# Runki2018/litehandnet

Hardware: AMD Instinct MI355X
Metric: images/sec fwd+bwd @256x256 bs64 litehandnet (higher is better)
Workload: dtype f32; 1 GPU; litehandnet variant B (MSRB hourglass litehourglass.py) C=128, 256x256x3 -> 21x64x64, per-GPU batch 64, train-mode BN, fwd + TopdownHeatmapLoss + bwd + fused Adam; global_batch=64, parallelism=dp1

## Files before the change

### litehandnet_amd/csrc/k_conv_stem.hip

```cpp
#include "lhn_common.h"

__global__ void __launch_bounds__(256) k_stem_fwd(const float* __restrict__ img, const float* __restrict__ w, lhn_view y,
                                                  double* __restrict__ stats, int Hi, int Wi, int K, int stride, int pad,
                                                  lhn_bnfin fin) {
  extern __shared__ __attribute__((aligned(16))) float smem[];
  const int CO = y.C, CG = CO >> 3, KK = K * K, T = 3 * KK;
  float* Ws = smem;
  float* red = smem + T * CO;
  const int tid = threadIdx.x;
  for (int i = tid; i < T * CO; i += 256) {
    const int co = i / T, t = i - co * T;
    Ws[t * CO + co] = w[i];
  }
  __syncthreads();
  const int cg = tid % CG, pl = tid / CG, PL = 256 / CG;
  const int64_t total = (int64_t)y.N * y.H * y.W;
  float s[8], q[8];
#pragma unroll
  for (int j = 0; j < 8; ++j) s[j] = q[j] = 0.f;
  for (int64_t pix = (int64_t)blockIdx.x * PL + pl; pix < total; pix += (int64_t)gridDim.x * PL) {
    const int wo = (int)(pix % y.W);
    const int64_t t = pix / y.W;
    const int ho = (int)(t % y.H), n = (int)(t / y.H);
    float acc[8];
#pragma unroll
    for (int j = 0; j < 8; ++j) acc[j] = 0.f;
    for (int c = 0; c < 3; ++c) {
      const float* plane = img + ((int64_t)n * 3 + c) * Hi * Wi;
      for (int kh = 0; kh < K; ++kh) {
        const int ih = ho * stride - pad + kh;
        if (ih < 0 || ih >= Hi) continue;
        for (int kw = 0; kw < K; ++kw) {
          const int iw = wo * stride - pad + kw;
          if (iw < 0 || iw >= Wi) continue;
          const float v = plane[(int64_t)ih * Wi + iw];
          const float* wr = Ws + (c * KK + kh * K + kw) * CO + cg * 8;
          const f4 w0 = *reinterpret_cast<const f4*>(wr), w1 = *reinterpret_cast<const f4*>(wr + 4);
          acc[0] += v * w0.x; acc[1] += v * w0.y; acc[2] += v * w0.z; acc[3] += v * w0.w;
          acc[4] += v * w1.x; acc[5] += v * w1.y; acc[6] += v * w1.z; acc[7] += v * w1.w;
        }
      }
    }
    float* o = y.data + pix * y.cstride + y.coff + cg * 8;
    *reinterpret_cast<f4*>(o) = (f4){acc[0], acc[1], acc[2], acc[3]};
    *reinterpret_cast<f4*>(o + 4) = (f4){acc[4], acc[5], acc[6], acc[7]};
#pragma unroll
    for (int j = 0; j < 8; ++j) {
      s[j] += acc[j];
      q[j] += acc[j] * acc[j];
    }
  }
  if (stats) {
#pragma unroll
    for (int j = 0; j < 8; ++j) {
      red[tid * 16 + j] = s[j];
      red[tid * 16 + 8 + j] = q[j];
    }
    __syncthreads();
    if (tid < CO) {
      const int g = tid >> 3, j = tid & 7;
      double sd = 0, qd = 0;
      for (int p = 0; p < PL; ++p) {
        sd += red[(p * CG + g) * 16 + j];
        qd += red[(p * CG + g) * 16 + 8 + j];
      }
      double* st = stats + (size_t)(blockIdx.x % LHN_STAT_REPLICAS) * 2 * CO;
      atomicAdd(st + tid, sd);
      atomicAdd(st + CO + tid, qd);
    }
    if (fin.counter && lhn_last_block(fin.counter)) lhn_bn_finalize_block(fin, stats);
  }
}


__global__ void __launch_bounds__(256) k_stem3_fwd_mfma(const float* __restrict__ img, const float* __restrict__ w, lhn_view y,
                                                        double* __restrict__ stats, int Hi, int Wi, int stride, int pad, lhn_bnfin fin) {
  constexpr int CO = 32, LDV = 36;
  __shared__ __attribute__((aligned(16))) float Vs[256 * LDV];
  __shared__ double redd[4][2 * CO];
  const int tid = threadIdx.x, lane = tid & 63, wave = __builtin_amdgcn_readfirstlane(tid >> 6), l31 = lane & 31, lh = lane >> 5;
  float wreg[16];
#pragma unroll
  for (int ks = 0; ks < 16; ++ks) {
    const int tap = 16 * lh + ks;
    wreg[ks] = tap < 27 ? w[l31 * 27 + tap] : 0.f;
  }
  for (int t = 27; t < 32; ++t) Vs[tid * LDV + t] = 0.f;
  const int64_t total = (int64_t)y.N * y.H * y.W;
  const int64_t ntiles = (total + 255) / 256;
  float v[27];
  auto issue = [&](int64_t tile) __attribute__((always_inline)) {
    const int64_t pix = tile * 256 + tid;
    const int64_t pc = pix < total ? pix : total - 1;
    const int wo = (int)(pc % y.W);
    const int64_t r = pc / y.W;
    const int ho = (int)(r % y.H), n = (int)(r / y.H);
#pragma unroll
    for (int c = 0; c < 3; ++c) {
      const float* plane = img + ((int64_t)n * 3 + c) * Hi * Wi;
#pragma unroll
      for (int kh = 0; kh < 3; ++kh) {
        const int ih = ho * stride - pad + kh, ihc = min(max(ih, 0), Hi - 1);
#pragma unroll
        for (int kw = 0; kw < 3; ++kw) {
          const int iw = wo * stride - pad + kw, iwc = min(max(iw, 0), Wi - 1);
          const float t = plane[(int64_t)ihc * Wi + iwc];
          v[c * 9 + kh * 3 + kw] = (ih == ihc && iw == iwc) ? t : 0.f;
        }
      }
    }
  };
  float s = 0.f, q = 0.f, kk = 0.f;
  int cnt = 0;
  int64_t tile = blockIdx.x;
  if (tile < ntiles) issue(tile);
  for (; tile < ntiles; tile += gridDim.x) {
    __syncthreads();
#pragma unroll
    for (int t = 0; t < 27; ++t) Vs[tid * LDV + t] = v[t];
    __syncthreads();
    if (tile + gridDim.x < ntiles) issue(tile + gridDim.x);
#pragma unroll
    for (int h = 0; h < 2; ++h) {
      const int prow = wave * 64 + 32 * h;
      const f4* ap = reinterpret_cast<const f4*>(Vs + (prow + l31) * LDV + 16 * lh);
      const f4 a0 = ap[0], a1 = ap[1], a2 = ap[2], a3 = ap[3];
      const float a[16] = {a0.x, a0.y, a0.z, a0.w, a1.x, a1.y, a1.z, a1.w, a2.x, a2.y, a2.z, a2.w, a3.x, a3.y, a3.z, a3.w};
      f16v acc;
#pragma unroll
      for (int r = 0; r < 16; ++r) acc[r] = 0.f;
#pragma unroll
      for (int ks = 0; ks < 16; ++ks) acc = __builtin_amdgcn_mfma_f32_32x32x2f32(a[ks], wreg[ks], acc, 0, 0, 0);
      const int64_t pbase = tile * 256 + prow + 4 * lh;
#pragma unroll
      for (int r = 0; r < 16; ++r) {
        const int64_t pix = pbase + (r & 3) + 8 * (r >> 2);
        if (pix < total) {
          y.data[pix * y.cstride + y.coff + l31] = acc[r];
          if (cnt == 0) kk = acc[r];
          const float d = acc[r] - kk;
          s += d;
          q += d * d;
          ++cnt;
        }
      }
    }
  }
  if (stats) {
    const double k0 = kk, c0 = cnt;
    double sd = (double)s + c0 * k0, qd = (double)q + 2.0 * k0 * (double)s + c0 * k0 * k0;
    sd += __shfl_xor(sd, 32, 64);
    qd += __shfl_xor(qd, 32, 64);
    if (lh == 0) {
      redd[wave][l31] = sd;
      redd[wave][CO + l31] = qd;
    }
    __syncthreads();
    if (tid < 2 * CO) {
      double* st = stats + (size_t)(blockIdx.x % LHN_STAT_REPLICAS) * 2 * CO;
      atomicAdd(st + tid, redd[0][tid] + redd[1][tid] + redd[2][tid] + redd[3][tid]);
    }
    if (fin.counter && lhn_last_block(fin.counter)) lhn_bn_finalize_block(fin, stats);
  }
}


__global__ void __launch_bounds__(256, 2) k_stem7_fwd_mfma(const float* __restrict__ img, const float* __restrict__ w, lhn_view y,
                                                        double* __restrict__ stats, int Hi, int Wi, int stride, int pad, lhn_bnfin fin) {
  constexpr int CO = 64, T = 147, TP = 160, NKS = TP / 2, LDV = TP + 4, BMP = 64, G = 4, NR = 6, NV = NR * 7;
  extern __shared__ __attribute__((aligned(16))) float smem[];
  float* Vs = smem;
  double* redd = reinterpret_cast<double*>(smem + BMP * LDV);
  const int tid = threadIdx.x, lane = tid & 63, wave = __builtin_amdgcn_readfirstlane(tid >> 6), l31 = lane & 31, lh = lane >> 5;
  const int cot = wave & 1, pg = wave >> 1, co = cot * 32 + l31;
  float wreg[NKS];
#pragma unroll
  for (int ks = 0; ks < NKS; ++ks) {
    const int tap = NKS * lh + ks;
    wreg[ks] = tap < T ? w[co * T + tap] : 0.f;
  }
  const int p = tid & (BMP - 1), g = tid >> 6;
  for (int t = T + g; t < TP; t += G) Vs[p * LDV + t] = 0.f;
  const int64_t total = (int64_t)y.N * y.H * y.W;
  const int64_t ntiles = (total + BMP - 1) / BMP;
  float v[NV];
  auto issue = [&](int64_t tile) __attribute__((always_inline)) {
    const int64_t pix = tile * BMP + p;
    const int64_t pc = pix < total ? pix : total - 1;
    const int wo = (int)(pc % y.W);
    const int64_t r = pc / y.W;
    const int ho = (int)(r % y.H), n = (int)(r / y.H);
    const float* base = img + (int64_t)n * 3 * Hi * Wi;
    const int iw0 = wo * stride - pad;
#pragma unroll
    for (int jr = 0; jr < NR; ++jr) {
      const int row = min(g + G * jr, 20), c = row / 7, kh = row - 7 * c;
      const int ih = ho * stride - pad + kh, ihc = min(max(ih, 0), Hi - 1);
      const float* rb = base + ((int64_t)c * Hi + ihc) * Wi;
#pragma unroll
      for (int kw = 0; kw < 7; ++kw) {
        const int iw = iw0 + kw, iwc = min(max(iw, 0), Wi - 1);
        const float q = rb[iwc];
        v[jr * 7 + kw] = (ih == ihc && iw == iwc) ? q : 0.f;
      }
    }
  };
  float s = 0.f, q = 0.f, kk = 0.f;
  int cnt = 0;
  int64_t tile = blockIdx.x;
  if (tile < ntiles) issue(tile);
  for (; tile < ntiles; tile += gridDim.x) {
    __syncthreads();
#pragma unroll
    for (int jr = 0; jr < NR; ++jr)
      if (g + G * jr < 21)
#pragma unroll
        for (int kw = 0; kw < 7; ++kw) Vs[p * LDV + (g + G * jr) * 7 + kw] = v[jr * 7 + kw];
    __syncthreads();
    if (tile + gridDim.x < ntiles) issue(tile + gridDim.x);
    const f4* ap = reinterpret_cast<const f4*>(Vs + (pg * 32 + l31) * LDV + NKS * lh);
    f16v acc;
#pragma unroll
    for (int r = 0; r < 16; ++r) acc[r] = 0.f;
#pragma unroll
    for (int c = 0; c < NKS / 4; ++c) {
      if ((c & 3) == 0) asm volatile("" ::: "memory");
      const f4 a = ap[c];
      acc = __builtin_amdgcn_mfma_f32_32x32x2f32(a.x, wreg[4 * c + 0], acc, 0, 0, 0);
      acc = __builtin_amdgcn_mfma_f32_32x32x2f32(a.y, wreg[4 * c + 1], acc, 0, 0, 0);
      acc = __builtin_amdgcn_mfma_f32_32x32x2f32(a.z, wreg[4 * c + 2], acc, 0, 0, 0);
      acc = __builtin_amdgcn_mfma_f32_32x32x2f32(a.w, wreg[4 * c + 3], acc, 0, 0, 0);
    }
    const int64_t pbase = tile * BMP + pg * 32 + 4 * lh;
#pragma unroll
    for (int r = 0; r < 16; ++r) {
      const int64_t pix = pbase + (r & 3) + 8 * (r >> 2);
      if (pix < total) {
        y.data[pix * y.cstride + y.coff + co] = acc[r];
        if (cnt == 0) kk = acc[r];
        const float d = acc[r] - kk;
        s += d;
        q += d * d;
        ++cnt;
      }
    }
  }
  if (stats) {
    const double k0 = kk, c0 = cnt;
    double sd = (double)s + c0 * k0, qd = (double)q + 2.0 * k0 * (double)s + c0 * k0 * k0;
    sd += __shfl_xor(sd, 32, 64);
    qd += __shfl_xor(qd, 32, 64);
    __syncthreads();
    if (lh == 0) {
      redd[pg * 2 * CO + co] = sd;
      redd[pg * 2 * CO + CO + co] = qd;
    }
    __syncthreads();
    if (tid < 2 * CO) {
      double* st = stats + (size_t)(blockIdx.x % LHN_STAT_REPLICAS) * 2 * CO;
      atomicAdd(st + tid, redd[tid] + redd[2 * CO + tid]);
    }
    if (fin.counter && lhn_last_block(fin.counter)) lhn_bn_finalize_block(fin, stats);
  }
}

extern "C" int lhn_conv_stem_fwd(const float* img, const float* w, const lhn_view* y, double* stats, int Hi, int Wi, int k,
                                 int stride, int pad, const lhn_bnfin* finp, void* stream) {
  lhn_bnfin fin;
  if (finp && stats) fin = *finp; else fin.counter = nullptr;
  LHN_CHECK_ARG(img && w && lhn_view_ok(y), "lhn_conv_stem_fwd: bad view / null pointer");
  LHN_CHECK_ARG(y->C % 8 == 0 && pow2(y->C / 8) && y->C <= 256, "lhn_conv_stem_fwd: Cout=%d", y->C);
  LHN_CHECK_ARG((k == 1 || k == 3 || k == 5 || k == 7) && stride >= 1, "lhn_conv_stem_fwd: k=%d", k);
  const int Ho = (Hi + 2 * pad - k) / stride + 1, Wo = (Wi + 2 * pad - k) / stride + 1;
  LHN_CHECK_ARG(y->H == Ho && y->W == Wo, "lhn_conv_stem_fwd: output %dx%d, expected %dx%d", y->H, y->W, Ho, Wo);
  const int PL = 256 / (y->C / 8);
  const size_t lds = (size_t)(3 * k * k * y->C) * 4 + 256 * 16 * 4;
  const bool mfma = !lhn_dw_force_gather() && ((k == 7 && y->C == 64) || (k == 3 && y->C == 32));
  LHN_CHECK_ARG(mfma || lds <= 65536, "lhn_conv_stem_fwd: k=%d Cout=%d needs %zu B of LDS (limit 65536 B)", k, y->C, lds);
  if (k == 7 && y->C == 64 && !lhn_dw_force_gather()) {
    const size_t lds7 = (size_t)64 * 164 * 4 + 2 * 2 * 64 * 8;
    static LhnKernelCfg cfg7;
    int per_cu = 1;
    if (!lhn_kernel_cfg(cfg7, &k_stem7_fwd_mfma, lds7, 3, &per_cu)) {
      lhn_set_error("lhn_conv_stem_fwd: cannot reserve %zu B of LDS", lds7);
      return 2;
    }
    const int64_t ntiles = ((int64_t)y->N * Ho * Wo + 63) / 64;
    int grid = lhn_num_cus() * per_cu;
    if (grid > ntiles) grid = (int)ntiles;
    hipLaunchKernelGGL(k_stem7_fwd_mfma, dim3(grid), dim3(256), lds7, (hipStream_t)stream, img, w, *y, stats, Hi, Wi, stride, pad, fin);
  } else if (k == 3 && y->C == 32 && !lhn_dw_force_gather()) {
    hipLaunchKernelGGL(k_stem3_fwd_mfma, dim3(grid_for((int64_t)y->N * Ho * Wo, 256, 3)), dim3(256), 0, (hipStream_t)stream, img, w, *y,
                       stats, Hi, Wi, stride, pad, fin);
  } else
    hipLaunchKernelGGL(k_stem_fwd, dim3(grid_for((int64_t)y->N * Ho * Wo, PL, 8)), dim3(256), lds, (hipStream_t)stream, img,
                       w, *y, stats, Hi, Wi, k, stride, pad, fin);
  LHN_CHECK_LAUNCH("lhn_conv_stem_fwd");
  return 0;
}

__device__ __forceinline__ f4 dw_load_dy(const lhn_view& y, const lhn_gradview& g, const Xf4& xf, const Gr4& gr,
                                         int64_t pix, int n, int h, int w, int ca) {
  const f4 raw = *reinterpret_cast<const f4*>(y.data + pix * y.cstride + ca);
  const f4 dz = *reinterpret_cast<const f4*>(g.dz + pix * y.cstride + ca);
  const f4 du = lhn_grad_du(y, g, xf, raw, dz, n, h, w, ca);
  return gr.A * du + gr.B * raw + gr.Cc;
}

template <int K, int KR>
__global__ void __launch_bounds__(256) k_stem_bwd(const float* __restrict__ img, lhn_view y, lhn_gradview gy,
                                                  float* __restrict__ dw, int Hi, int Wi, int stride, int pad, int nrep,
                                                  int64_t rep_stride, int kh0) {
  dw += (size_t)(blockIdx.x % nrep) * rep_stride;
  constexpr int T = 3 * KR * K;
  __shared__ f4 red[256];
  const int C4 = y.C >> 2;
  const int tid = threadIdx.x, c4 = tid % C4, pl = tid / C4, PL = 256 / C4;
  const int cy = y.coff + 4 * c4;
  const Xf4 yxf = lhn_load_xf(y, cy);
  const Gr4 ygr = lhn_load_coef(gy, y.cstride, cy);
  f4 acc[T];
#pragma unroll
  for (int i = 0; i < T; ++i) acc[i] = (f4){0.f, 0.f, 0.f, 0.f};
  const int64_t total = (int64_t)y.N * y.H * y.W;
  for (int64_t pix = (int64_t)blockIdx.x * PL + pl; pix < total; pix += (int64_t)gridDim.x * PL) {
    const int wo = (int)(pix % y.W);
    const int64_t t = pix / y.W;
    const int ho = (int)(t % y.H), n = (int)(t / y.H);
    const f4 dy = dw_load_dy(y, gy, yxf, ygr, pix, n, ho, wo, cy);
#pragma unroll
    for (int c = 0; c < 3; ++c) {
      const float* plane = img + ((int64_t)n * 3 + c) * Hi * Wi;
#pragma unroll
      for (int r = 0; r < KR; ++r) {
        const int ih = ho * stride - pad + kh0 + r;
#pragma unroll
        for (int kw = 0; kw < K; ++kw) {
          const int iw = wo * stride - pad + kw;
          float v = 0.f;
          if (ih >= 0 && ih < Hi && iw >= 0 && iw < Wi) v = plane[(int64_t)ih * Wi + iw];
          acc[(c * KR + r) * K + kw] += dy * v;
        }
      }
    }
  }
  constexpr int TW = 3 * K * K;
#pragma unroll
  for (int i = 0; i < T; ++i) {
    __syncthreads();
    red[tid] = acc[i];
    __syncthreads();
    if (tid < C4) {
      f4 s = (f4){0.f, 0.f, 0.f, 0.f};
      for (int j = 0; j < PL; ++j) s += red[j * C4 + tid];
      const int c = i / (KR * K), r = (i / K) % KR, kw = i % K, e = c * K * K + (kh0 + r) * K + kw;
      atomicAdd(dw + (4 * tid + 0) * TW + e, s.x);
      atomicAdd(dw + (4 * tid + 1) * TW + e, s.y);
      atomicAdd(dw + (4 * tid + 2) * TW + e, s.z);
      atomicAdd(dw + (4 * tid + 3) * TW + e, s.w);
    }
  }
}


__global__ void __launch_bounds__(256) k_stem3_bwd_mfma(const float* __restrict__ img, lhn_view y, lhn_gradview gy, float* __restrict__ dw,
                                                        int Hi, int Wi, int stride, int pad, int nrep, int64_t rep_stride) {
  constexpr int CO = 32, LDY = CO + 4, LDV = 33;
  extern __shared__ __attribute__((aligned(16))) float smem[];
  float* dYs = smem;
  float* Vs = smem + 256 * LDY;
  const int tid = threadIdx.x, lane = tid & 63, wave = __builtin_amdgcn_readfirstlane(tid >> 6), l31 = lane & 31, lh = lane >> 5;
  const int c4 = tid & 7, prow = tid >> 3;
  const int cy = y.coff + 4 * c4;
  const Xf4 yxf = lhn_load_xf(y, cy);
  const Gr4 ygr = lhn_load_coef(gy, y.cstride, cy);
  for (int t = 27; t < 32; ++t) Vs[tid * LDV + t] = 0.f;
  f16v acc;
#pragma unroll
  for (int r = 0; r < 16; ++r) acc[r] = 0.f;
  const int64_t total = (int64_t)y.N * y.H * y.W;
  const int64_t ntiles = (total + 255) / 256;
  f4 yraw[8], zraw[8];
  float v[27];
  auto issue = [&](int64_t tile) __attribute__((always_inline)) {
#pragma unroll
    for (int j = 0; j < 8; ++j) {
      int64_t pix = tile * 256 + prow + 32 * j;
      pix = pix < total ? pix : total - 1;
      yraw[j] = *reinterpret_cast<const f4*>(y.data + pix * y.cstride + cy);
      zraw[j] = *reinterpret_cast<const f4*>(gy.dz + pix * y.cstride + cy);
    }
    const int64_t pix = tile * 256 + tid;
    const int64_t pc = pix < total ? pix : total - 1;
    const int wo = (int)(pc % y.W);
    const int64_t r = pc / y.W;
    const int ho = (int)(r % y.H), n = (int)(r / y.H);
#pragma unroll
    for (int c = 0; c < 3; ++c) {
      const float* plane = img + ((int64_t)n * 3 + c) * Hi * Wi;
#pragma unroll
      for (int kh = 0; kh < 3; ++kh) {
        const int ih = ho * stride - pad + kh, ihc = min(max(ih, 0), Hi - 1);
#pragma unroll
        for (int kw = 0; kw < 3; ++kw) {
          const int iw = wo * stride - pad + kw, iwc = min(max(iw, 0), Wi - 1);
          const float t = plane[(int64_t)ihc * Wi + iwc];
          v[c * 9 + kh * 3 + kw] = (ih == ihc && iw == iwc) ? t : 0.f;
        }
      }
    }
  };
  int64_t tile = blockIdx.x;
  if (tile < ntiles) issue(tile);
  for (; tile < ntiles; tile += gridDim.x) {
    __syncthreads();
#pragma unroll
    for (int j = 0; j < 8; ++j) {
      const int p = prow + 32 * j;
      const int64_t pix = tile * 256 + p;
      f4 d = (f4){0.f, 0.f, 0.f, 0.f};
      if (pix < total) {
        const int wo = (int)(pix % y.W);
        const int64_t r = pix / y.W;
        const f4 du = lhn_grad_du(y, gy, yxf, yraw[j], zraw[j], (int)(r / y.H), (int)(r % y.H), wo, cy);
        d = ygr.A * du + ygr.B * yraw[j] + ygr.Cc;
      }
      *reinterpret_cast<f4*>(dYs + p * LDY + 4 * c4) = d;
    }
#pragma unroll
    for (int t = 0; t < 27; ++t) Vs[tid * LDV + t] = v[t];
    __syncthreads();
    if (tile + gridDim.x < ntiles) issue(tile + gridDim.x);
    const float* ar = dYs + (wave * 64 + lh) * LDY + l31;
    const float* br = Vs + (wave * 64 + lh) * LDV + l31;
#pragma unroll 8
    for (int ks = 0; ks < 32; ++ks) acc = __builtin_amdgcn_mfma_f32_32x32x2f32(ar[2 * ks * LDY], br[2 * ks * LDV], acc, 0, 0, 0);
  }
  __syncthreads();
  float* part = dYs;
#pragma unroll
  for (int r = 0; r < 16; ++r) part[(wave * 16 + r) * 64 + lane] = acc[r];
  __syncthreads();
  dw += (size_t)(blockIdx.x % nrep) * rep_stride;
  for (int i = tid; i < CO * 27; i += 256) {
    const int co = i / 27, t = i - co * 27;
    const int r = (co & 3) + 4 * (co >> 3), ln = t + 32 * ((co >> 2) & 1);
    const float v = part[(0 * 16 + r) * 64 + ln] + part[(1 * 16 + r) * 64 + ln] + part[(2 * 16 + r) * 64 + ln] + part[(3 * 16 + r) * 64 + ln];
    atomicAdd(dw + i, v);
  }
}


__global__ void __launch_bounds__(256, 2) k_stem7_bwd_mfma(const float* __restrict__ img, lhn_view y, lhn_gradview gy, float* __restrict__ dw,
                                                           int Hi, int Wi, int stride, int pad, int nrep, int64_t rep_stride) {
  constexpr int CO = 64, T = 147, LDY = CO + 4, LDV = 161, BMP = 64, G = 4, NR = 6;
  extern __shared__ __attribute__((aligned(16))) float smem[];
  float* dYs = smem;
  float* Vs = smem + BMP * LDY;
  const int tid = threadIdx.x, lane = tid & 63, wave = __builtin_amdgcn_readfirstlane(tid >> 6), l31 = lane & 31, lh = lane >> 5;
  const int c4 = tid & 15, prow = tid >> 4;
  const int cy = y.coff + 4 * c4;
  const Xf4 yxf = lhn_load_xf(y, cy);
  const Gr4 ygr = lhn_load_coef(gy, y.cstride, cy);
  const int p = tid & (BMP - 1), g = tid >> 6;
  for (int t = T + g; t < 160; t += G) Vs[p * LDV + t] = 0.f;
  f16v acc[3];
#pragma unroll
  for (int i = 0; i < 3; ++i)
#pragma unroll
    for (int r = 0; r < 16; ++r) acc[i][r] = 0.f;
  const int64_t total = (int64_t)y.N * y.H * y.W;
  const int64_t ntiles = (total + BMP - 1) / BMP;
  f4 yraw[4], zraw[4];
  float v[NR * 7];
  auto issue = [&](int64_t tile) __attribute__((always_inline)) {
#pragma unroll
    for (int j = 0; j < 4; ++j) {
      int64_t pix = tile * BMP + prow + 16 * j;
      pix = pix < total ? pix : total - 1;
      yraw[j] = *reinterpret_cast<const f4*>(y.data + pix * y.cstride + cy);
      zraw[j] = *reinterpret_cast<const f4*>(gy.dz + pix * y.cstride + cy);
    }
    const int64_t pix = tile * BMP + p;
    const int64_t pc = pix < total ? pix : total - 1;
    const int wo = (int)(pc % y.W);
    const int64_t r = pc / y.W;
    const int ho = (int)(r % y.H), n = (int)(r / y.H);
    const float* base = img + (int64_t)n * 3 * Hi * Wi;
    const int iw0 = wo * stride - pad;
#pragma unroll
    for (int jr = 0; jr < NR; ++jr) {
      const int row = min(g + G * jr, 20), c = row / 7, kh = row - 7 * c;
      const int ih = ho * stride - pad + kh, ihc = min(max(ih, 0), Hi - 1);
      const float* rb = base + ((int64_t)c * Hi + ihc) * Wi;
#pragma unroll
      for (int kw = 0; kw < 7; ++kw) {
        const int iw = iw0 + kw, iwc = min(max(iw, 0), Wi - 1);
        const float q = rb[iwc];
        v[jr * 7 + kw] = (ih == ihc && iw == iwc) ? q : 0.f;
      }
    }
  };
  int64_t tile = blockIdx.x;
  if (tile < ntiles) issue(tile);
  for (; tile < ntiles; tile += gridDim.x) {
    __syncthreads();
#pragma unroll
    for (int j = 0; j < 4; ++j) {
      const int pp = prow + 16 * j;
      const int64_t pix = tile * BMP + pp;
      f4 d = (f4){0.f, 0.f, 0.f, 0.f};
      if (pix < total) {
        const int wo = (int)(pix % y.W);
        const int64_t r = pix / y.W;
        const f4 du = lhn_grad_du(y, gy, yxf, yraw[j], zraw[j], (int)(r / y.H), (int)(r % y.H), wo, cy);
        d = ygr.A * du + ygr.B * yraw[j] + ygr.Cc;
      }
      *reinterpret_cast<f4*>(dYs + pp * LDY + 4 * c4) = d;
    }
#pragma unroll
    for (int jr = 0; jr < NR; ++jr)
      if (g + G * jr < 21)
#pragma unroll
        for (int kw = 0; kw < 7; ++kw) Vs[p * LDV + (g + G * jr) * 7 + kw] = v[jr * 7 + kw];
    __syncthreads();
    if (tile + gridDim.x < ntiles) issue(tile + gridDim.x);
#pragma unroll
    for (int i = 0; i < 3; ++i) {
      const int job = wave + 4 * i;
      if (job < 10) {
        const float* ar = dYs + lh * LDY + (job & 1) * 32 + l31;
        const float* br = Vs + lh * LDV + (job >> 1) * 32 + l31;
#pragma unroll 8
        for (int ks = 0; ks < 32; ++ks) acc[i] = __builtin_amdgcn_mfma_f32_32x32x2f32(ar[2 * ks * LDY], br[2 * ks * LDV], acc[i], 0, 0, 0);
      }
    }
  }
  dw += (size_t)(blockIdx.x % nrep) * rep_stride;
#pragma unroll
  for (int i = 0; i < 3; ++i) {
    const int job = wave + 4 * i;
    if (job < 10) {
      const int t = (job >> 1) * 32 + l31;
#pragma unroll
      for (int r = 0; r < 16; ++r) {
        const int co = (job & 1) * 32 + (r & 3) + 8 * (r >> 2) + 4 * lh;
        if (t < T) atomicAdd(dw + co * T + t, acc[i][r]);
      }
    }
  }
}

extern "C" int lhn_conv_stem_bwd(const float* img, const lhn_view* y, const lhn_gradview* gy, float* dw, int Hi, int Wi, int k,
                                 int stride, int pad, int nrep, int64_t rep_stride, void* stream) {
  if (nrep < 1) nrep = 1;
  LHN_CHECK_ARG(img && lhn_view_ok(y) && gy && gy->dz && dw, "lhn_conv_stem_bwd: bad view / null pointer");
  LHN_CHECK_ARG(pow2(y->C / 4) && y->C <= 256 && (k == 1 || k == 3 || k == 7), "lhn_conv_stem_bwd: Cout=%d k=%d", y->C, k);
  const int PL = 256 / (y->C / 4);
  const int g = grid_for((int64_t)y->N * y->H * y->W, PL, 4);
  if (k == 7 && y->C == 64 && !lhn_dw_force_gather()) {
    const size_t lds = (size_t)64 * (68 + 161) * 4;
    static LhnKernelCfg cfg7;
    int per_cu = 1;
    if (!lhn_kernel_cfg(cfg7, &k_stem7_bwd_mfma, lds, 2, &per_cu)) {
      lhn_set_error("lhn_conv_stem_bwd: cannot reserve %zu B of LDS", lds);
      return 2;
    }
    const int64_t ntiles = ((int64_t)y->N * y->H * y->W + 63) / 64;
    int grid = lhn_num_cus() * per_cu;
    if (grid > ntiles) grid = (int)ntiles;
    hipLaunchKernelGGL(k_stem7_bwd_mfma, dim3(grid), dim3(256), lds, (hipStream_t)stream, img, *y, *gy, dw, Hi, Wi, stride, pad, nrep, rep_stride);
  } else if (k == 3 && y->C == 32 && !lhn_dw_force_gather()) {
    const size_t lds = (size_t)256 * (36 + 33) * 4;
    static LhnKernelCfg cfg;
    int per_cu = 1;
    if (!lhn_kernel_cfg(cfg, &k_stem3_bwd_mfma, lds, 2, &per_cu)) {
      lhn_set_error("lhn_conv_stem_bwd: cannot reserve %zu B of LDS", lds);
      return 2;
    }
    const int64_t ntiles = ((int64_t)y->N * y->H * y->W + 255) / 256;
    int grid = lhn_num_cus() * per_cu;
    if (grid > ntiles) grid = (int)ntiles;
    hipLaunchKernelGGL(k_stem3_bwd_mfma, dim3(grid), dim3(256), lds, (hipStream_t)stream, img, *y, *gy, dw, Hi, Wi, stride, pad, nrep, rep_stride);
  } else if (k == 3)
    hipLaunchKernelGGL((k_stem_bwd<3, 3>), dim3(g), dim3(256), 0, (hipStream_t)stream, img, *y, *gy, dw, Hi, Wi, stride, pad, nrep, rep_stride, 0);
  else if (k == 1)
    hipLaunchKernelGGL((k_stem_bwd<1, 1>), dim3(g), dim3(256), 0, (hipStream_t)stream, img, *y, *gy, dw, Hi, Wi, stride, pad, nrep, rep_stride, 0);
  else
    for (int kh = 0; kh < 7; ++kh)
      hipLaunchKernelGGL((k_stem_bwd<7, 1>), dim3(g), dim3(256), 0, (hipStream_t)stream, img, *y, *gy, dw, Hi, Wi, stride, pad, nrep, rep_stride, kh);
  LHN_CHECK_LAUNCH("lhn_conv_stem_bwd");
  return 0;
}
```

Baseline: 9508 images/s.

## Add per-wave tiled stem3 conv fwd/bwd kernels with double-buffered gathers

Adds new 3x3 stem conv forward and backward MFMA kernels in which each wave owns 32-pixel tiles. Image gathers are double-buffered in registers and prefetched while the current tile's MFMAs run, and pixel indices are advanced incrementally instead of recomputed with divisions. The backward kernel uses per-wave LDS slices with wave barriers instead of block-wide syncs, and has a template variant that skips gate/pool index math when those are absent. The path is on by default, can be disabled with an env var, and is limited to inputs under 2^30 elements because offsets are 32-bit.

```diff
diff --git a/litehandnet_amd/csrc/k_conv_stem.hip b/litehandnet_amd/csrc/k_conv_stem.hip
--- a/litehandnet_amd/csrc/k_conv_stem.hip
+++ b/litehandnet_amd/csrc/k_conv_stem.hip
@@ -145,6 +145,149 @@
         }
       }
     }
+  }
+  if (stats) {
+    const double k0 = kk, c0 = cnt;
+    double sd = (double)s + c0 * k0, qd = (double)q + 2.0 * k0 * (double)s + c0 * k0 * k0;
+    sd += __shfl_xor(sd, 32, 64);
+    qd += __shfl_xor(qd, 32, 64);
+    if (lh == 0) {
+      redd[wave][l31] = sd;
+      redd[wave][CO + l31] = qd;
+    }
+    __syncthreads();
+    if (tid < 2 * CO) {
+      double* st = stats + (size_t)(blockIdx.x % LHN_STAT_REPLICAS) * 2 * CO;
+      atomicAdd(st + tid, redd[0][tid] + redd[1][tid] + redd[2][tid] + redd[3][tid]);
+    }
+    if (fin.counter && lhn_last_block(fin.counter)) lhn_bn_finalize_block(fin, stats);
+  }
+}
+
+
+struct Stem3Pix {
+  int n, ho, wo, dn[2], dh[2], dw[2];
+  __device__ __forceinline__ void init(int64_t p, int64_t step0, int64_t step1, int H, int W) {
+    wo = (int)(p % W);
+    int64_t r = p / W;
+    ho = (int)(r % H), n = (int)(r / H);
+    dw[0] = (int)(step0 % W);
+    r = step0 / W;
+    dh[0] = (int)(r % H), dn[0] = (int)(r / H);
+    dw[1] = (int)(step1 % W);
+    r = step1 / W;
+    dh[1] = (int)(r % H), dn[1] = (int)(r / H);
+  }
+  __device__ __forceinline__ void advance(int H, int W, int i) {
+    wo += dw[i];
+    int c = wo >= W;
+    wo -= c ? W : 0;
+    ho += dh[i] + c;
+    c = ho >= H;
+    ho -= c ? H : 0;
+    n += dn[i] + c;
+  }
+};
+__device__ __forceinline__ void stem3_gather(const float* __restrict__ img, int n, int ho, int wo, int lh, int Hi, int Wi, int stride,
+                                             int pad, float (&v)[16], unsigned& mask) {
+  const int HW = Hi * Wi, base = n * 3 * HW;
+  int ro[3], cl[3];
+  unsigned rok = 0, cok = 0;
+#pragma unroll
+  for (int k = 0; k < 3; ++k) {
+    const int ih = ho * stride - pad + k, ihc = min(max(ih, 0), Hi - 1);
+    const int iw = wo * stride - pad + k, iwc = min(max(iw, 0), Wi - 1);
+    ro[k] = ihc * Wi;
+    cl[k] = iwc;
+    rok |= (unsigned)(ih == ihc) << k;
+    cok |= (unsigned)(iw == iwc) << k;
+  }
+  unsigned m = 0;
+#pragma unroll
+  for (int ks = 0; ks < 16; ++ks) {
+    const int t0 = ks, t1 = 16 + ks < 27 ? 16 + ks : ks;
+    const int o0 = (t0 / 9) * HW + ro[(t0 % 9) / 3] + cl[t0 % 3], o1 = (t1 / 9) * HW + ro[(t1 % 9) / 3] + cl[t1 % 3];
+    const unsigned k0 = (rok >> ((t0 % 9) / 3)) & (cok >> (t0 % 3)) & 1u;
+    const unsigned k1 = 16 + ks < 27 ? ((rok >> ((t1 % 9) / 3)) & (cok >> (t1 % 3)) & 1u) : 0u;
+    v[ks] = *reinterpret_cast<const float*>(reinterpret_cast<const char*>(img) + (unsigned)(base + (lh ? o1 : o0)) * 4u);
+    m |= (lh ? k1 : k0) << ks;
+  }
+  mask = m;
+}
+static bool stem3_wave_tiles_on(int N, int Hi, int Wi) {
+  static int v = -1;
+  if (v < 0) {
+    const char* e = getenv("LHN_STEM3_WAVE_TILES");
+    v = (e && e[0] == '0') ? 0 : 1;
+  }
+  return v != 0 && (int64_t)N * 3 * Hi * Wi < ((int64_t)1 << 30);
+}
+
+__global__ void __launch_bounds__(256, 4) k_stem3_fwd_mfma_wt(const float* __restrict__ img, const float* __restrict__ w, lhn_view y,
+                                                           double* __restrict__ stats, int Hi, int Wi, int stride, int pad, lhn_bnfin fin) {
+  constexpr int CO = 32;
+  __shared__ double redd[4][2 * CO];
+  const int tid = threadIdx.x, lane = tid & 63, wave = __builtin_amdgcn_readfirstlane(tid >> 6), l31 = lane & 31, lh = lane >> 5;
+  float wreg[16];
+#pragma unroll
+  for (int ks = 0; ks < 16; ++ks) {
+    const int tap = 16 * lh + ks;
+    wreg[ks] = tap < 27 ? w[l31 * 27 + tap] : 0.f;
+  }
+  const int64_t total = (int64_t)y.N * y.H * y.W;
+  const int64_t nblk = (total + 255) / 256, G = gridDim.x;
+  Stem3Pix px;
+  px.init(((int64_t)blockIdx.x * 8 + 2 * wave) * 32 + l31, 32, (8 * G - 1) * 32, y.H, y.W);
+  float va[16], vb[16];
+  unsigned ma = 0, mb = 0;
+  auto issue = [&](float (&v)[16], unsigned& m, int second) __attribute__((always_inline)) {
+    stem3_gather(img, min(px.n, y.N - 1), px.ho, px.wo, lh, Hi, Wi, stride, pad, v, m);
+    px.advance(y.H, y.W, second);
+  };
+  float s = 0.f, q = 0.f, kk = 0.f;
+  int cnt = 0;
+  const unsigned voff = (unsigned)(4 * lh * y.cstride + l31) * 4u;
+  auto tile_of = [&](float (&v)[16], unsigned& m, int64_t tile, bool more, int second) __attribute__((always_inline)) {
+    f16v acc;
+#pragma unroll
+    for (int r = 0; r < 16; ++r) acc[r] = 0.f;
+#pragma unroll
+    for (int ks = 0; ks < 16; ++ks) acc = __builtin_amdgcn_mfma_f32_32x32x2f32(((m >> ks) & 1u) ? v[ks] : 0.f, wreg[ks], acc, 0, 0, 0);
+    if (more) issue(v, m, second);
+    char* const ybase = reinterpret_cast<char*>(y.data + tile * 32 * y.cstride + y.coff);
+    const int left = (int)max((int64_t)0, min((int64_t)32, total - tile * 32));
+    if (left == 32) {
+#pragma unroll
+      for (int r = 0; r < 16; ++r) {
+        *reinterpret_cast<float*>(ybase + (size_t)((r & 3) + 8 * (r >> 2)) * y.cstride * 4 + voff) = acc[r];
+        if (cnt == 0) kk = acc[r];
+        const float d = acc[r] - kk;
+        s += d;
+        q += d * d;
+        ++cnt;
+      }
+    } else {
+#pragma unroll
+      for (int r = 0; r < 16; ++r)
+        if (4 * lh + (r & 3) + 8 * (r >> 2) < left) {
+          *reinterpret_cast<float*>(ybase + (size_t)((r & 3) + 8 * (r >> 2)) * y.cstride * 4 + voff) = acc[r];
+          if (cnt == 0) kk = acc[r];
+          const float d = acc[r] - kk;
+          s += d;
+          q += d * d;
+          ++cnt;
+        }
+    }
+  };
+  int64_t T = blockIdx.x;
+  if (T < nblk) {
+    issue(va, ma, 0);
+    issue(vb, mb, 1);
+  }
+  for (; T < nblk; T += G) {
+    const bool more = T + G < nblk;
+    tile_of(va, ma, T * 8 + 2 * wave, more, 0);
+    tile_of(vb, mb, T * 8 + 2 * wave + 1, more, 1);
   }
   if (stats) {
     const double k0 = kk, c0 = cnt;
@@ -290,8 +433,12 @@
     if (grid > ntiles) grid = (int)ntiles;
     hipLaunchKernelGGL(k_stem7_fwd_mfma, dim3(grid), dim3(256), lds7, (hipStream_t)stream, img, w, *y, stats, Hi, Wi, stride, pad, fin);
   } else if (k == 3 && y->C == 32 && !lhn_dw_force_gather()) {
-    hipLaunchKernelGGL(k_stem3_fwd_mfma, dim3(grid_for((int64_t)y->N * Ho * Wo, 256, 3)), dim3(256), 0, (hipStream_t)stream, img, w, *y,
-                       stats, Hi, Wi, stride, pad, fin);
+    if (stem3_wave_tiles_on(y->N, Hi, Wi)) {
+      hipLaunchKernelGGL(k_stem3_fwd_mfma_wt, dim3(grid_for((int64_t)y->N * Ho * Wo, 256, 3)), dim3(256), 0, (hipStream_t)stream, img, w, *y,
+                         stats, Hi, Wi, stride, pad, fin);
+    } else
+      hipLaunchKernelGGL(k_stem3_fwd_mfma, dim3(grid_for((int64_t)y->N * Ho * Wo, 256, 3)), dim3(256), 0, (hipStream_t)stream, img, w, *y,
+                         stats, Hi, Wi, stride, pad, fin);
   } else
     hipLaunchKernelGGL(k_stem_fwd, dim3(grid_for((int64_t)y->N * Ho * Wo, PL, 8)), dim3(256), lds, (hipStream_t)stream, img,
                        w, *y, stats, Hi, Wi, k, stride, pad, fin);
@@ -438,6 +585,103 @@
   }
   __syncthreads();
   float* part = dYs;
+#pragma unroll
+  for (int r = 0; r < 16; ++r) part[(wave * 16 + r) * 64 + lane] = acc[r];
+  __syncthreads();
+  dw += (size_t)(blockIdx.x % nrep) * rep_stride;
+  for (int i = tid; i < CO * 27; i += 256) {
+    const int co = i / 27, t = i - co * 27;
+    const int r = (co & 3) + 4 * (co >> 3), ln = t + 32 * ((co >> 2) & 1);
+    const float v = part[(0 * 16 + r) * 64 + ln] + part[(1 * 16 + r) * 64 + ln] + part[(2 * 16 + r) * 64 + ln] + part[(3 * 16 + r) * 64 + ln];
+    atomicAdd(dw + i, v);
+  }
+}
+
+
+template <bool GP>
+__global__ void __launch_bounds__(256, 2) k_stem3_bwd_mfma_wt(const float* __restrict__ img, lhn_view y, lhn_gradview gy, float* __restrict__ dw,
+                                                           int Hi, int Wi, int stride, int pad, int nrep, int64_t rep_stride) {
+  if constexpr (!GP) {
+    y.gate = nullptr;
+    gy.dpool = nullptr;
+  }
+  constexpr int CO = 32, LDY = CO + 4, LDV = 33, WS = 32 * (LDY + LDV);
+  extern __shared__ __attribute__((aligned(16))) float smem[];
+  const int tid = threadIdx.x, lane = tid & 63, wave = __builtin_amdgcn_readfirstlane(tid >> 6), l31 = lane & 31, lh = lane >> 5;
+  float* dYs = smem + wave * WS;
+  float* Vs = dYs + 32 * LDY;
+  const int c4 = lane & 7, prow = lane >> 3;
+  const int cy = y.coff + 4 * c4;
+  const Xf4 yxf = lhn_load_xf(y, cy);
+  const Gr4 ygr = lhn_load_coef(gy, y.cstride, cy);
+  f16v acc;
+#pragma unroll
+  for (int r = 0; r < 16; ++r) acc[r] = 0.f;
+  const int64_t total = (int64_t)y.N * y.H * y.W;
+  const int64_t nblk = (total + 255) / 256, G = gridDim.x;
+  Stem3Pix px;
+  px.init(((int64_t)blockIdx.x * 8 + 2 * wave) * 32 + l31, 32, (8 * G - 1) * 32, y.H, y.W);
+  f4 ya[4], za[4], yb[4], zb[4];
+  float va[16], vb[16];
+  unsigned ma = 0, mb = 0;
+  auto issue = [&](int64_t tile, f4 (&yr)[4], f4 (&zr)[4], float (&v)[16], unsigned& m, int second) __attribute__((always_inline)) {
+    const int64_t p0 = min(tile * 32, total - 1);
+    const char* const yp = reinterpret_cast<const char*>(y.data + p0 * y.cstride);
+    const char* const zp = reinterpret_cast<const char*>(gy.dz + p0 * y.cstride);
+    const int last = (int)min((int64_t)31, total - 1 - p0);
+#pragma unroll
+    for (int j = 0; j < 4; ++j) {
+      const unsigned off = (unsigned)(min(prow + 8 * j, last) * y.cstride + cy) * 4u;
+      yr[j] = *reinterpret_cast<const f4*>(yp + off);
+      zr[j] = *reinterpret_cast<const f4*>(zp + off);
+    }
+    stem3_gather(img, min(px.n, y.N - 1), px.ho, px.wo, lh, Hi, Wi, stride, pad, v, m);
+    px.advance(y.H, y.W, second);
+  };
+  auto tile_of = [&](int64_t tile, f4 (&yr)[4], f4 (&zr)[4], float (&v)[16], unsigned& m, bool more, int second) __attribute__((always_inline)) {
+#pragma unroll
+    for (int j = 0; j < 4; ++j) {
+      const int p = prow + 8 * j;
+      const int64_t pix = tile * 32 + p;
+      f4 d = (f4){0.f, 0.f, 0.f, 0.f};
+      if (pix < total) {
+        int n = 0, h = 0, wo = 0;
+        if constexpr (GP) {
+          wo = (int)(pix % y.W);
+          const int64_t r = pix / y.W;
+          h = (int)(r % y.H), n = (int)(r / y.H);
+        }
+        const f4 du = lhn_grad_du(y, gy, yxf, yr[j], zr[j], n, h, wo, cy);
+        d = ygr.A * du + ygr.B * yr[j] + ygr.Cc;
+      }
+      *reinterpret_cast<f4*>(dYs + p * LDY + 4 * c4) = d;
+    }
+#pragma unroll
+    for (int ks = 0; ks < 16; ++ks) Vs[l31 * LDV + 16 * lh + ks] = ((m >> ks) & 1u) ? v[ks] : 0.f;
+    __builtin_amdgcn_fence(__ATOMIC_RELEASE, "wavefront");
+    __builtin_amdgcn_wave_barrier();
+    __builtin_amdgcn_fence(__ATOMIC_ACQUIRE, "wavefront");
+    if (more) issue(tile + 8 * G, yr, zr, v, m, second);
+    const float* ar = dYs + lh * LDY + l31;
+    const float* br = Vs + lh * LDV + l31;
+#pragma unroll
+    for (int ks = 0; ks < 16; ++ks) acc = __builtin_amdgcn_mfma_f32_32x32x2f32(ar[2 * ks * LDY], br[2 * ks * LDV], acc, 0, 0, 0);
+    __builtin_amdgcn_fence(__ATOMIC_RELEASE, "wavefront");
+    __builtin_amdgcn_wave_barrier();
+    __builtin_amdgcn_fence(__ATOMIC_ACQUIRE, "wavefront");
+  };
+  int64_t T = blockIdx.x;
+  if (T < nblk) {
+    issue(T * 8 + 2 * wave, ya, za, va, ma, 0);
+    issue(T * 8 + 2 * wave + 1, yb, zb, vb, mb, 1);
+  }
+  for (; T < nblk; T += G) {
+    const bool more = T + G < nblk;
+    tile_of(T * 8 + 2 * wave, ya, za, va, ma, more, 0);
+    tile_of(T * 8 + 2 * wave + 1, yb, zb, vb, mb, more, 1);
+  }
+  __syncthreads();
+  float* part = smem;
 #pragma unroll
   for (int r = 0; r < 16; ++r) part[(wave * 16 + r) * 64 + lane] = acc[r];
   __syncthreads();
@@ -571,17 +815,28 @@
     if (grid > ntiles) grid = (int)ntiles;
     hipLaunchKernelGGL(k_stem7_bwd_mfma, dim3(grid), dim3(256), lds, (hipStream_t)stream, img, *y, *gy, dw, Hi, Wi, stride, pad, nrep, rep_stride);
   } else if (k == 3 && y->C == 32 && !lhn_dw_force_gather()) {
-    const size_t lds = (size_t)256 * (36 + 33) * 4;
-    static LhnKernelCfg cfg;
+    const bool wt = stem3_wave_tiles_on(y->N, Hi, Wi);
+    const size_t lds = wt ? (size_t)4 * 32 * (36 + 33) * 4 : (size_t)256 * (36 + 33) * 4;
+    static LhnKernelCfg cfg, cfgw;
     int per_cu = 1;
-    if (!lhn_kernel_cfg(cfg, &k_stem3_bwd_mfma, lds, 2, &per_cu)) {
+    const bool gp = y->gate || gy->dpool;
+    static LhnKernelCfg cfgp;
+    if (!(wt ? (gp ? lhn_kernel_cfg(cfgp, &k_stem3_bwd_mfma_wt<true>, lds, 2, &per_cu) : lhn_kernel_cfg(cfgw, &k_stem3_bwd_mfma_wt<false>, lds, 2, &per_cu))
+             : lhn_kernel_cfg(cfg, &k_stem3_bwd_mfma, lds, 2, &per_cu))) {
       lhn_set_error("lhn_conv_stem_bwd: cannot reserve %zu B of LDS", lds);
       return 2;
     }
     const int64_t ntiles = ((int64_t)y->N * y->H * y->W + 255) / 256;
     int grid = lhn_num_cus() * per_cu;
     if (grid > ntiles) grid = (int)ntiles;
-    hipLaunchKernelGGL(k_stem3_bwd_mfma, dim3(grid), dim3(256), lds, (hipStream_t)stream, img, *y, *gy, dw, Hi, Wi, stride, pad, nrep, rep_stride);
+    if (wt) {
+      if (gp)
+        hipLaunchKernelGGL(k_stem3_bwd_mfma_wt<true>, dim3(grid), dim3(256), lds, (hipStream_t)stream, img, *y, *gy, dw, Hi, Wi, stride, pad, nrep, rep_stride);
+      else
+        hipLaunchKernelGGL(k_stem3_bwd_mfma_wt<false>, dim3(grid), dim3(256), lds, (hipStream_t)stream, img, *y, *gy, dw, Hi, Wi, stride, pad, nrep, rep_stride);
+    } else {
+      hipLaunchKernelGGL(k_stem3_bwd_mfma, dim3(grid), dim3(256), lds, (hipStream_t)stream, img, *y, *gy, dw, Hi, Wi, stride, pad, nrep, rep_stride);
+    }
   } else if (k == 3)
     hipLaunchKernelGGL((k_stem_bwd<3, 3>), dim3(g), dim3(256), 0, (hipStream_t)stream, img, *y, *gy, dw, Hi, Wi, stride, pad, nrep, rep_stride, 0);
   else if (k == 1)
```

After: 9594 images/s (median of 6 runs). No clear change (+0.9%).
